# YukunXia/VLOAM-CMU-16833

Measured on AMD Instinct MI355X. Metric: scans/sec end-to-end odometry on 64x2048 cloud, higher is better.
Workload: dtype f32 points / f64 poses+residuals; 1 GPU; configs[2]: scanRegistration + laserOdometry + laserMapping scan-to-map ICP (voxel-hash local map, ~200 scans), synthetic HDL-64E 64x2048; sequences=1, map_warmup_sweeps=200, map_points_at_last_sweep=119454

## Files before the change

### vloam-cmu-16833_amd/csrc/map_inspect.hip

```cpp
#include <hip/hip_runtime.h>
#include <string.h>
#include <vector>
#include "map_kernels.h"

namespace vloam {

__global__ void k_map_error_fetch(MapFrame* fr, int clear_mask, int* out) { out[0] = atomicAnd(&fr->error, ~clear_mask); out[1] = fr->fallback_solves; }

vloam_status map_error(MapContext* m, int* e, int clear_mask, long long* fallback_solves) {
  *e = 0;
  if (fallback_solves) *fallback_solves = 0;
  for (int b = 0; b < m->se.B; b++) {
    const MapContext mb = m->for_session(b);
    int* d_out = mb.rebuild_n;
    VL_RAW_LAUNCH(k_map_error_fetch, dim3(1), dim3(1), 0, 0, mb.frame, clear_mask, d_out);
    int v[2] = {0, 0};
    if (hipMemcpy(v, d_out, sizeof(v), hipMemcpyDeviceToHost) != hipSuccess) return VLOAM_ERR_HIP;
    *e |= v[0];
    if (fallback_solves) *fallback_solves += v[1];
  }
  return VLOAM_OK;
}

vloam_status map_debug_get(MapContext* m0, int item, void* buf, long long cap, long long* n) {
  const MapContext msel = m0->for_session(m0->sel);
  const MapContext* m = &msel;
  if (item == 64) return copy_dev(m->state, sizeof(MapState), buf, cap, n);
  if (item == 65) return copy_dev(m->frame, sizeof(MapFrame), buf, cap, n);
  if (item == 66) return copy_dev(m->cube_cnt, sizeof(int) * 2 * kCubeNum, buf, cap, n);
  if (item == 67 || item == 68) {
    const VoxelTable& T = m->tab[item - 67];
    const size_t slots = (size_t)T.mask + 1;
    std::vector<VoxelRec> recs(slots);
    if (hipMemcpy(recs.data(), T.rec, slots * sizeof(VoxelRec), hipMemcpyDeviceToHost) != hipSuccess) return VLOAM_ERR_HIP;
    std::vector<unsigned> rows;
    for (size_t s = 0; s < slots; s++) {
      if (recs[s].key == 0 || recs[s].count == 0) continue;
      if ((recs[s].key >> 56) == 0 && (recs[s].count & (1 << 30))) continue;
      unsigned r[7];
      r[0] = (unsigned)(recs[s].key & 0xffffffffu); r[1] = (unsigned)(recs[s].key >> 32); r[2] = (unsigned)recs[s].count;
      memcpy(r + 3, &recs[s].sx, 16);
      rows.insert(rows.end(), r, r + 7);
    }
    if (n) *n = (long long)(rows.size() * 4);
    const size_t c = rows.size() * 4 < (size_t)cap ? rows.size() * 4 : (size_t)cap;
    if (buf && c) memcpy(buf, rows.data(), c);
    return VLOAM_OK;
  }
  if (item == 72) return copy_dev(m->ts_log, sizeof(long long) * 2048, buf, cap, n);
  if (item == 73) return copy_dev(m->cbox, sizeof(int4) * 2 * (size_t)m->factor_cap(), buf, cap, n);
  if (item == 71) return copy_dev(m->assoc_cyc, sizeof(long long) * 16, buf, cap, n);
  if (item == 69) {
    int out[12] = {0};
    for (int k = 0; k < 2; k++) if (hipMemcpy(out + 4 * k, m->tab[k].stats, 4 * sizeof(int), hipMemcpyDeviceToHost) != hipSuccess) return VLOAM_ERR_HIP;
    MapFrame fr;
    if (hipMemcpy(&fr, m->frame, sizeof(fr), hipMemcpyDeviceToHost) != hipSuccess) return VLOAM_ERR_HIP;
    out[8] = (int)m0->rebuilds; out[9] = fr.max_candidates; out[10] = fr.n_deferred[0] + fr.n_newraw[0]; out[11] = fr.n_deferred[1] + fr.n_newraw[1];
    if (n) *n = sizeof(out);
    if (buf) memcpy(buf, out, (size_t)cap < sizeof(out) ? (size_t)cap : sizeof(out));
    return VLOAM_OK;
  }
  const int outer = item / 16, k = item % 16;
  if (outer < 0 || outer > 1) return VLOAM_ERR_INVALID;
  const FactorTable& F = m->F[outer];
  switch (k) {
    case 0: return copy_dev(F.type, sizeof(int) * F.cap, buf, cap, n);
    case 1: return copy_dev(F.A, sizeof(double) * 3 * F.cap, buf, cap, n);
    case 2: return copy_dev(F.B, sizeof(double) * 3 * F.cap, buf, cap, n);
    case 3: return copy_dev(m->rec + outer, sizeof(LMRecord), buf, cap, n);
    case 4: return copy_dev(F.resid, sizeof(double) * 3 * F.cap, buf, cap, n);
    case 5: return copy_dev(F.p, sizeof(double) * 3 * F.cap, buf, cap, n);
  }
  return VLOAM_ERR_INVALID;
}

vloam_status map_counts(MapContext* m0, long long c[16]) {
  const MapContext msel = m0->for_session(m0->sel);
  const MapContext* m = &msel;
  MapState ms;
  MapFrame fr;
  LMRecord rec[2];
  if (hipMemcpy(&ms, m->state, sizeof(ms), hipMemcpyDeviceToHost) != hipSuccess) return VLOAM_ERR_HIP;
  if (hipMemcpy(&fr, m->frame, sizeof(fr), hipMemcpyDeviceToHost) != hipSuccess) return VLOAM_ERR_HIP;
  if (hipMemcpy(rec, m->rec, sizeof(rec), hipMemcpyDeviceToHost) != hipSuccess) return VLOAM_ERR_HIP;
  c[11] = ms.n_corner_stack; c[12] = ms.n_surf_stack;
  c[13] = fr.n_factors[1][0] + fr.n_factors[1][1];
  c[14] = ms.do_optimize ? (long long)(rec[0].n_evals + rec[1].n_evals) : 0;
  c[15] = ms.n_map_corner + ms.n_map_surf;
  return VLOAM_OK;
}

}
```

### vloam-cmu-16833_amd/csrc/map_kernels.h

```cpp
#pragma once
#include <hip/hip_runtime.h>
#include <vector>
#include "../../include/vloam_hip/c_api.h"
#include "sr_kernels.h"
#include "vloam_device.h"

namespace vloam {

constexpr int kCubeW = 21, kCubeH = 21, kCubeD = 11, kCubeNum = kCubeW * kCubeH * kCubeD;
constexpr int kStackCapCorner = 8192;
constexpr int kStackCapSurf = 24576;
constexpr int kMapFactorCap = kStackCapCorner + kStackCapSurf;
constexpr int kStackCapSurfStep = 8192, kStackCapSurfMax = 131072;
static_assert(kStackCapSurfMax <= (1 << 17), "the tier's raw-point arrival stamp keeps 17 bits of stack index (k_map_finalize_tier)");
constexpr int kPendCap = 16;
__host__ __device__ inline int vox_radix(float inv) { return (int)(50.0f * inv) + 4; }

struct __attribute__((aligned(32))) VoxelRec {
  unsigned long long key;
  float sx, sy, sz, si;
  int count;
  int pend_cnt;
};
static_assert(sizeof(VoxelRec) == 32, "one voxel, one half cache line");
// ... 67 lines not shown
  float4* out[2] = {nullptr, nullptr};
  PubHeader* hdr[2] = {nullptr, nullptr};
  float4* cloud[2] = {nullptr, nullptr};
  int* cloud_n[2] = {nullptr, nullptr};
  hipEvent_t ev_map[2] = {nullptr, nullptr}, ev_cloud[2] = {nullptr, nullptr};
  int map_seq = 0, cloud_seq = 0;
  int map_frame[2] = {-1, -1}, cloud_frame[2] = {-1, -1};
  int mapped = 0;
  void rebase(size_t o) {
    rbp(cnt, o); rbp(off, o); rbp(cur, o); rbp(keys, o); rbp(vals, o);
    for (int k = 0; k < 2; k++) { rbp(out[k], o); rbp(hdr[k], o); rbp(cloud[k], o); rbp(cloud_n[k], o); }
  }
};

struct MapGrow {
  int max_log2 = 28;
  int lg[2] = {0, 0};
  long long steps = 0;
  long long inc_rec[2] = {0, 0};
  long long inc_blk[2] = {0, 0};
  unsigned long long* progress = nullptr;
  long long step_at[2] = {-1, -1};
  static constexpr int kEvRing = 4;
  hipEvent_t ev_prog[kEvRing] = {};
  int failed_log2 = 0;
  struct Retired { void* p[3]; hipEvent_t ev; };
  std::vector<Retired> retired;
  std::vector<void*> leftover;
};

struct LocAux { int shift[3]; int si_error; double guess[7]; };
struct MapLocalize {
  char* base = nullptr;
  MapState* state = nullptr;
  MapFrame* frame = nullptr;
  LocAux* aux = nullptr;
  StackInfo* si = nullptr;
  FrameScalars* S = nullptr;
  float4* in[2] = {nullptr, nullptr};
  float4* stack[2] = {nullptr, nullptr};
  DsScratch ds[2];
  unsigned ds_gen = 0;
  FactorTable F[2];
  LMRecord* rec = nullptr;
  float4* nbr = nullptr;
  int4* cbox = nullptr;
  float4* ccand = nullptr;
  vloam_localize_result* result = nullptr;
};

struct CarveGeom {
  int rows, cols, n_sweeps, min_votes;
  float min_range, max_range, range_res;
  float elev_min, row_scale, col_scale;
  unsigned margin_q;
};
struct CarvePose { double R[9], t[3]; };
constexpr int kCarveMaxSweeps = 16, kCarveMaxPoints = 262144, kCarveMaxPixels = 1 << 20;
constexpr int kCarveCounters = 6;
struct CarveCounters { unsigned long long cnt[2][kCarveCounters]; unsigned long long n_removed; };
struct MapCarve { char* base = nullptr; size_t bytes = 0; };
struct MergeXf { double R[9], t[3]; int identity; };

struct MapArchive {
  char* base = nullptr;
  int* cnt = nullptr;
  vloam_map_archive_row* rows = nullptr;
  long long cap = 0;
  int frame = 0;
};

struct MapContext {
  MapState* state = nullptr;
  MapFrame* frame = nullptr;
  VoxelTable tab[2];
  int* cube_cnt = nullptr;
  DsScratch ds[2];
  unsigned ds_gen = 0;
  static constexpr int kSets = kBufferSets;
  float4* stack_sets[kSets][2] = {};
  StackInfo* stack_info[kSets] = {};
  float4* stack[2] = {nullptr, nullptr};
  float4* stack_map[2] = {nullptr, nullptr};
  int* touched[2] = {nullptr, nullptr};
  int* deferred[2] = {nullptr, nullptr};
  int* newraw[2] = {nullptr, nullptr};
  FactorTable F[2];
  LMRecord* rec = nullptr;
  int surf_cap = kStackCapSurf;
  int factor_cap() const { return kStackCapCorner + surf_cap; }
  bool tier() const { return surf_cap > kStackCapSurf; }
  float4* nbr = nullptr;
  int4* cbox = nullptr;
  float4* ccand = nullptr;
  VoxelRec* rebuild_tmp = nullptr;
  int rebuild_cap = 0;
  int* rebuild_n = nullptr;
  int* host_flags = nullptr;
  int rebuild_cooldown[kMaxBatch][2] = {};
  long long rebuilds = 0;
  MapGrow* grow = nullptr;
  Sess se;
  int sel = 0;
  MapContext for_session(int b) const {
    MapContext m = *this;
    const size_t off = (size_t)b * se.ss;
    rbp(m.state, off); rbp(m.frame, off); m.tab[0].rebase(off); m.tab[1].rebase(off); rbp(m.cube_cnt, off); m.ds[0].rebase(off); m.ds[1].rebase(off);
    for (int c = 0; c < kSets; c++) { rbp(m.stack_sets[c][0], off); rbp(m.stack_sets[c][1], off); rbp(m.stack_info[c], off); }
    for (int k = 0; k < 2; k++) { rbp(m.stack[k], off); rbp(m.stack_map[k], off); rbp(m.touched[k], off); rbp(m.deferred[k], off); rbp(m.newraw[k], off); m.F[k].rebase(off); }
    rbp(m.rec, off); rbp(m.nbr, off); rbp(m.cbox, off); rbp(m.ccand, off); rbp(m.registered, off); rbp(m.assoc_cyc, off); rbp(m.ts_log, off); rbp(m.rebuild_tmp, off); rbp(m.rebuild_n, off);
    if (m.host_flags) m.host_flags += 2 * b;
    m.pub.rebase(off);
    m.se.B = 1; m.sel = 0;
    return m;
  }
  MapLocalize* loc = nullptr;
  MapCarve* carve = nullptr;
  MapArchive* archive = nullptr;
  MapPub pub;
  float4* registered = nullptr;
  long long* assoc_cyc = nullptr;
  long long* ts_log = nullptr;
  int max_points = 0;
  float inv_leaf[2] = {0, 0};
};

vloam_status map_layout(MapContext* m, const vloam_config& cfg, Arena& A);
vloam_status map_init(MapContext* m, hipStream_t st);
vloam_status map_enqueue(MapContext* m, const vloam_config& cfg, hipStream_t st, const SRBuffers& cur, LOState* lo, double* traj_row14,
                         bool skip_frame, int set, ProfHook* ph, hipEvent_t done = nullptr);
vloam_status map_force_rebuild(MapContext* m, hipStream_t st);
vloam_status map_reclaim_enqueue(MapContext* m, hipStream_t st, int kind);
void map_destroy(MapContext* m);
vloam_status map_stack_enqueue(MapContext* m, hipStream_t st, const SRBuffers& cur, int set, ProfHook* ph, hipEvent_t done = nullptr);
vloam_status map_get_cloud(MapContext* m, hipStream_t st, int which, const SRBuffers& cur, float* xyzi4, int cap, int* n);
vloam_status map_export(MapContext* m, hipStream_t st, float* xyzi4, long long cap, long long* n);
vloam_status map_export_kind(MapContext* m, hipStream_t st, int kind, float* xyzi4, long long cap, long long* n);
bool map_publishes(const MapContext* m, bool skip_frame);
vloam_status map_publish_enqueue(MapContext* m, hipStream_t st, const float4* cloud, const FrameScalars* S, int frame, bool skip_frame, ProfHook* ph,
                                 hipEvent_t done);
vloam_status map_published_get(MapContext* m, int which, float* xyzi4, long long cap, long long* n, int* frame, void** d_ptr);
vloam_status map_error(MapContext* m, int* err_bits, int clear_mask = 0, long long* fallback_solves = nullptr);
vloam_status map_debug_get(MapContext* m, int item, void* buf, long long cap, long long* n);
vloam_status map_counts(MapContext* m, long long c[16]);
vloam_status map_query_enqueue(MapContext* m, hipStream_t st, int kind, int k, float radius, const void* d_xyz_pad4, int n, void* d_xyzi4, void* d_d2,
                               void* d_count);
vloam_status map_score_enqueue(MapContext* m, hipStream_t st, const void* d_corner, int n_corner, const void* d_surf, int n_surf, const int stride[2],
                               const float radius[2], const double* d_q4t3, int M, void* d_out);
vloam_status map_localize_alloc(MapContext* m, hipStream_t st);
void map_localize_free(MapContext* m);
vloam_status map_localize_enqueue(MapContext* m, hipStream_t st, const float4* corner, int n_corner, const float4* surf, int n_surf, int set,
                                  const double* row7, const double pose7[7], int pose_frame, vloam_localize_result* d_result);
void map_loc_prepare_launch(hipStream_t st, const MapContext* m, const StackInfo* si, const double* row7, const double pose7[7], int pose_frame);
void map_loc_finish_launch(hipStream_t st, const MapContext* m, vloam_localize_result* d_result);
void map_stack_enqueue_loc(MapContext* m, hipStream_t st, const float4* corner, const float4* surf);
vloam_status map_import_run(MapContext* m, hipStream_t st, const double pose7[7], const void* const cloud[2], const int n[2], bool host_clouds,
                            vloam_map_import_result* h_result);
vloam_status map_merge_run(MapContext* m, hipStream_t st, const MergeXf& X, const void* const cloud[2], const int n[2], bool host_clouds, bool apply,
                           bool place_start, vloam_map_merge_result* h_result);
inline bool map_window_never_placed(const MapState& s) { return s.sweep_no == 0 && s.centerCube[0] == 0 && s.centerCube[1] == 0 && s.centerCube[2] == 0; }
vloam_status map_carve_run(MapContext* m, int session, hipStream_t st, const CarveGeom& G, int kind_mask, const void* const* clouds, const int* n,
                           const CarvePose* poses, bool host_io, void* removed, long long cap, bool apply, CarveCounters* h_out);
void map_carve_free(MapContext* m);
vloam_status map_archive_alloc(MapContext* m, hipStream_t st, long long capacity_rows);
void map_archive_free(MapContext* m);
void map_archive_enqueue(const MapContext* m, hipStream_t st);
vloam_status map_force_grow(MapContext* m, hipStream_t st);
void map_grow_release(MapContext* m);
vloam_status map_grow_init(MapContext* m, hipStream_t st);
void map_grow_destroy(MapContext* m);
vloam_status map_grow_rehash(MapContext* m, hipStream_t st, int kind);
vloam_status map_grow_before_sweep(MapContext* m, hipStream_t st);
void map_grow_progress_enqueue(MapContext* m, hipStream_t st);
vloam_status map_ckpt_pack(MapContext* m, hipStream_t st, long long n_rec[2], VoxelRec** d_out, float ms[2]);
vloam_status map_ckpt_unpack(MapContext* m, hipStream_t st, const void* recs, const long long n_rec[2], float* ms);
int map_grow_restore_log2(const MapContext* m, int kind, long long live, long long blk);
vloam_status map_grow_restore(MapContext* m, hipStream_t st, const int lg[2], const long long live[2], const long long blk[2], long long mapped);

}
```

### vloam-cmu-16833_amd/csrc/map_kernels.hip

```cpp
#include <hip/hip_runtime.h>
#include <math.h>
#include <string.h>
#include <type_traits>
#include "lm_solve.h"
#include "map_kernels.h"
#include "map_device.h"
#include "map_table.h"
#include "map_move_dev.h"
#include "subwave.h"

namespace vloam {

__device__ void map_purge(const VoxelTable& T, const MapState* ms, int first, int stride) {
  const int cW = ms->cenW, cH = ms->cenH, cD = ms->cenD;
  int dead = 0;
  for (unsigned s = (unsigned)first; s <= T.mask; s += (unsigned)stride) {
    const RecVal v = rec_load(&T.rec[s]);
    if (v.key == 0 || v.count == 0) continue;
    int Ai, Aj, Ak;
    unpack_cube(v.key, &Ai, &Aj, &Ak);
    const int i = Ai + cW, j = Aj + cH, kk = Ak + cD;
    if (i < 0 || i >= kCubeW || j < 0 || j >= kCubeH || kk < 0 || kk >= kCubeD) { rec_store_value(&T.rec[s], make_float4(0.f, 0.f, 0.f, 0.f), 0, 0); dead++; }
  }
  if (dead) atomicAdd(&T.stats[1], dead);
// ... 327 lines not shown
      float4 cc[U];
#pragma unroll
      for (int u = 0; u < U; u++) {
        const int w = c0 + gl + u * G;
        cc[u] = make_float4(0.f, 0.f, 0.f, __uint_as_float(0xffffffffu));
        if (from_cache && act && w < total) cc[u] = ccand[(size_t)slot * kCandCache + w];
      }
#pragma unroll
      for (int u = 0; u < U; u++) {
        const unsigned tie = __float_as_uint(cc[u].w);
        const float d0 = q0 - cc[u].x, d1 = q1 - cc[u].y, d2 = q2 - cc[u].z;
        const u64 k = ((u64)__float_as_uint(d0 * d0 + d1 * d1 + d2 * d2) << 32) | tie;
        if (from_cache && tie != 0xffffffffu) { key_u[u] = k; px[u] = cc[u].x; py[u] = cc[u].y; pz[u] = cc[u].z; }
      }
    }
    if (dbg_cyc && c0 == 0) tp[4] = clock64() + ((int)key_u[0] & 0);
    select_rounds(act, c0 > 0);
    if (dbg_cyc && c0 == 0) tp[5] = clock64();
  }
  const int nraw = min(s_nraw[qi], kRawCap);
  const bool raw_overflow = s_nraw[qi] > kRawCap;
  if (__ballot(live && nraw > 0) != 0ull) {
    int total_raw = 0;
    for (c0 = 0;; c0 += CH) {
      const bool act = live && nraw > 0 && (c0 == 0 || c0 < total_raw);
      if (__ballot(act) == 0ull) break;
      reset_candidates();
      int produced = 0;
      for (int r0 = 0; __ballot(act && r0 < nraw) != 0ull; r0 += G) {
        const int r = r0 + gl;
        const int nr = (act && r < nraw) ? s_rawn[qi][r] : 0;
        const u64 vk = (act && r < nraw) ? s_rawk[qi][r] : 0ull;
        const int inc = grp_scan_incl<G>(nr);
        const int tot = grp_sum<G>(nr);
        int o = produced + inc - nr;
        for (int j = 1; j <= nr; j++, o++)
          if (o >= c0 && o < c0 + CH) s_cand[qi][o - c0] = key_with_seq(vk, j);
        produced += tot;
      }
      if (act) total_raw = produced;
      sw_lds_sync();
      ncand = act ? min(total_raw - c0, CH) : 0;
      probe_pair(std::integral_constant<int, 0>{});
      if constexpr (U > 2) { if (__ballot(2 * G < ncand) != 0ull) probe_pair(std::integral_constant<int, 2>{}); }
      select_rounds(act, true);
    }
  }
  if (outer == 0 && search && gl == 0) {
    cbox[2 * slot] = make_int4(blo0, bhi0, blo1, bhi1);
    cbox[2 * slot + 1] = make_int4(blo2, bhi2, (total <= kCandCache && !overflow && s_nraw[qi] == 0) ? total : -1, total);
  }
  if (live && gl < 5) {
    const u64 k4 = s_bestk[qi][4];
    const bool ok = k4 != ~0ull && __uint_as_float((unsigned)(k4 >> 32)) < 1.0f;
    float4 p = s_bestp[qi][gl];
    p.w = ok ? 1.0f : 0.0f;
    nbr[slot * 5 + gl] = p;
  }
  if (live && gl == 0 && total > kCandChunk) atomicMax(&fr->max_candidates, total);
  if (__ballot(chain_too_long || (live && overflow)) && lane == 0) atomicOr(&fr->error, kErrMapFull);
  if (__ballot(live && raw_overflow) && lane == 0) atomicOr(&fr->error, kErrMapDeferred);
  if (dbg_cyc && lane == 0) {
    tp[6] = clock64();
    if (tp[3] == 0) tp[3] = tp[2];
    if (tp[4] == 0) tp[4] = tp[3];
    for (int k = 0; k < 6; k++) atomicAdd((unsigned long long*)&dbg_cyc[outer * 8 + k], (unsigned long long)(tp[k + 1] - tp[k]));
    atomicAdd((unsigned long long*)&dbg_cyc[outer * 8 + 7], 1ull);
  }
}

#define VL_MAP_TIER 0
#define VL_MAP_KERNEL(name) name
#define VL_MAP_CAP_PARAM
#define VL_MAP_SURF_CAP kStackCapSurf
#define VL_MAP_FACTOR_CAP kMapFactorCap
#include "map_prepare_fit.inc.h"
#define VL_MAP_TIER 1
#define VL_MAP_KERNEL(name) name##_tier
#define VL_MAP_CAP_PARAM , int surf_cap
#define VL_MAP_SURF_CAP surf_cap
#define VL_MAP_FACTOR_CAP F.cap
#include "map_prepare_fit.inc.h"

__device__ void map_update(MapState* ms, double* traj_row14) {
  const double* q = ms->q_wodom_curr;
  const double n2 = q[0] * q[0] + q[1] * q[1] + q[2] * q[2] + q[3] * q[3];
  double qi[4] = {0, 0, 0, 0};
  if (n2 > 0.0) { qi[0] = -q[0] / n2; qi[1] = -q[1] / n2; qi[2] = -q[2] / n2; qi[3] = q[3] / n2; }
  double r[4], t[3];
  dquat_mul(ms->parameters, qi, r);
  for (int k = 0; k < 4; k++) ms->q_wmap_wodom[k] = r[k];
  dquat_rot(ms->q_wmap_wodom, ms->t_wodom_curr, t);
  for (int k = 0; k < 3; k++) ms->t_wmap_wodom[k] = ms->parameters[4 + k] - t[k];
  if (traj_row14) for (int k = 0; k < 7; k++) traj_row14[7 + k] = ms->parameters[k];
}

__device__ bool map_put_raw_point(const VoxelTable& T, u64 voxel_key, int seq, float4 p, int stamp) {
  const u64 key = key_with_seq(voxel_key, seq);
  unsigned s = (unsigned)mix64(key) & T.mask;
  for (int probe = 0; probe < kMaxProbe; probe++, s = (s + 1) & T.mask) {
    const u64 old = atomicCAS(&T.rec[s].key, 0ull, key);
    if (old == 0ull || old == key) {
      if (old == 0ull) atomicAdd(&T.stats[0], 1);
      rec_store_value(&T.rec[s], p, 1, stamp);
      return true;
    }
  }
  return false;
}
__device__ void map_drop_raw_points(const VoxelTable& T, u64 voxel_key, int n) {
  int dead = 0;
  for (int seq = 1; seq <= min(n, 255); seq++) {
    const u64 key = key_with_seq(voxel_key, seq);
    unsigned s = (unsigned)mix64(key) & T.mask;
    for (int probe = 0; probe < kMaxProbe; probe++, s = (s + 1) & T.mask) {
      const u64 k = T.rec[s].key;
      if (k == 0ull) break;
      if (k == key) { rec_store_value(&T.rec[s], make_float4(0.f, 0.f, 0.f, 0.f), 0, 0); dead++; break; }
    }
  }
  if (dead) atomicAdd(&T.stats[1], dead);
}

template <bool TIER>
__device__ __forceinline__ void map_insert_body(const float4* __restrict__ stack0, const float4* __restrict__ stack1,
                                                float4* __restrict__ smap0, float4* __restrict__ smap1, VoxelTable T0, VoxelTable T1,
                                                float inv0, float inv1, MapState* ms, MapFrame* fr, int* __restrict__ touched0,
                                                int* __restrict__ touched1, int* __restrict__ deferred0, int* __restrict__ deferred1,
                                                double* traj_row14, size_t ss, int surf_cap) {
  VL_SESSION(ss); RB(stack0); RB(stack1); RB(smap0); RB(smap1); T0.rebase(so_); T1.rebase(so_); RB(ms); RB(fr); RB(touched0); RB(touched1);
  RB(deferred0); RB(deferred1); RB(traj_row14);
  if (blockIdx.x == 0 && blockIdx.y == 0 && threadIdx.x == 0) map_update(ms, traj_row14);
  const int kind = blockIdx.y;
  const VoxelTable T = kind ? T1 : T0;
  const float inv = kind ? inv1 : inv0;
  const float4* stack = kind ? stack1 : stack0;
  float4* smap = kind ? smap1 : smap0;
  int* touched = kind ? touched1 : touched0;
  (void)deferred0; (void)deferred1;
  const int n = kind ? ms->n_surf_stack : ms->n_corner_stack;
  const int cap = kind ? (TIER ? surf_cap : kStackCapSurf) : kStackCapCorner;
  const int lane = threadIdx.x & 63;
  const int i_first = blockIdx.x * 256 + threadIdx.x;
  const float4 p_first = stack[i_first < cap ? i_first : 0];
  for (int i0 = blockIdx.x * 256 + (threadIdx.x & ~63); i0 < n; i0 += gridDim.x * 256) {
    const int i = i0 + lane;
    auto insert_point = [&]() -> int {
      if (i >= n) return -1;
      const float4 p = associate_to_map(i == i_first ? p_first : stack[i], ms->parameters, ms->parameters + 4);
      smap[i] = p;
      const int Ai = cube_abs((double)p.x), Aj = cube_abs((double)p.y), Ak = cube_abs((double)p.z);
      const int wi = Ai + ms->cenW, wj = Aj + ms->cenH, wk = Ak + ms->cenD;
      if (wi < 0 || wi >= kCubeW || wj < 0 || wj >= kCubeH || wk < 0 || wk >= kCubeD) return -1;
      const int lx = (int)floorf(p.x * inv) - cube_voxel_base(Ai, inv), ly = (int)floorf(p.y * inv) - cube_voxel_base(Aj, inv),
                lz = (int)floorf(p.z * inv) - cube_voxel_base(Ak, inv);
      if ((unsigned)lx > (unsigned)kVoxMax || (unsigned)ly > (unsigned)kVoxMax || (unsigned)lz > (unsigned)kVoxMax || !cube_in_key_range(Ai, Aj, Ak)) { atomicOr(&fr->error, kErrMapFull); return -1; }
      const u64 key = pack_key(Ai, Aj, Ak, lx, ly, lz);
      unsigned s = (unsigned)mix64(key) & T.mask;
      for (int probe = 0; probe < kMaxProbe; probe++, s = (s + 1) & T.mask) {
        const u64 old = atomicCAS(&T.rec[s].key, 0ull, key);
        if (old == 0ull || old == key) {
          if (old == 0ull) {
            atomicAdd(&T.stats[0], 1);
            if (!map_publish_block(T, Ai, Aj, Ak, lx, ly, lz)) atomicOr(&fr->error, kErrMapFull);
          }
          const int pos = atomicAdd(&T.rec[s].pend_cnt, 1);
          if (pos < kPendCap) T.pend[(size_t)s * kPendCap + pos] = i; else atomicOr(&fr->error, kErrMapFull);
          return pos == 0 ? (int)s : -1;
        }
      }
      atomicOr(&fr->error, kErrMapFull);
      return -1;
    };
    const int first = insert_point();
    const u64 tm = __ballot(first >= 0);
    if (tm != 0ull) {
      const int leader = __ffsll((long long)tm) - 1;
      int base = 0;
      if (lane == leader) base = atomicAdd(&fr->n_touched[kind], __popcll(tm));
      base = __shfl(base, leader);
      if (first >= 0) {
        const int tpos = base + __popcll(tm & ((1ull << lane) - 1ull));
        if (tpos < cap) touched[tpos] = first; else atomicOr(&fr->error, kErrMapFull);
      }
    }
  }
}
#define VL_MAP_INSERT_PARAMS const float4* __restrict__ stack0, const float4* __restrict__ stack1, float4* __restrict__ smap0, float4* __restrict__ smap1, \
    VoxelTable T0, VoxelTable T1, float inv0, float inv1, MapState* ms, MapFrame* fr, int* __restrict__ touched0, int* __restrict__ touched1,      \
    int* __restrict__ deferred0, int* __restrict__ deferred1, double* traj_row14, size_t ss
#define VL_MAP_INSERT_ARGS stack0, stack1, smap0, smap1, T0, T1, inv0, inv1, ms, fr, touched0, touched1, deferred0, deferred1, traj_row14, ss
__global__ __launch_bounds__(256) void k_map_insert(VL_MAP_INSERT_PARAMS) { map_insert_body<false>(VL_MAP_INSERT_ARGS, kStackCapSurf); }
__global__ __launch_bounds__(256) void k_map_insert_tier(VL_MAP_INSERT_PARAMS, int surf_cap) { map_insert_body<true>(VL_MAP_INSERT_ARGS, surf_cap); }
#undef VL_MAP_INSERT_PARAMS
#undef VL_MAP_INSERT_ARGS

template <bool TIER>
__device__ __forceinline__ void map_finalize_body(const float4* __restrict__ smap0, const float4* __restrict__ smap1, VoxelTable T0,
                                                  VoxelTable T1, MapState* ms, MapFrame* fr,
                                                  const int* __restrict__ touched0, const int* __restrict__ touched1,
                                                  int* __restrict__ deferred0, int* __restrict__ deferred1, int* __restrict__ newraw0,
                                                  int* __restrict__ newraw1, int* __restrict__ cube_cnt, int* host_flags, long long* ts_log, size_t ss,
                                                  int surf_cap) {
  VL_SESSION(ss); RB(smap0); RB(smap1); T0.rebase(so_); T1.rebase(so_); RB(ms); RB(fr); RB(touched0); RB(touched1); RB(deferred0); RB(deferred1);
  RB(newraw0); RB(newraw1); RB(cube_cnt); RB(ts_log);
  if (ts_log && blockIdx.x == 0 && blockIdx.y == 0 && threadIdx.x == 0) ts_log[2 * ((ms->sweep_no - 1) & 1023) + 1] = (long long)wall_clock64();
  if (host_flags) host_flags += 2 * blockIdx.z;
  const int kind = blockIdx.y;
  const VoxelTable T = kind ? T1 : T0;
  const float4* smap = kind ? smap1 : smap0;
  const int* touched = kind ? touched1 : touched0;
  const int cap = kind ? (TIER ? surf_cap : kStackCapSurf) : kStackCapCorner;
  const int t = blockIdx.x * 256 + threadIdx.x;
  const int s_spec = touched[t < cap ? t : 0];
  const int nt = min(fr->n_touched[kind], cap);
  const int cI = ms->centerCube[0], cJ = ms->centerCube[1], cK = ms->centerCube[2];
  int* deferred = kind ? deferred1 : deferred0;
  int* newraw = kind ? newraw1 : newraw0;
  if (t < nt) {
    const int s = s_spec;
    int idx[kPendCap];
    const RecVal rv = rec_load(&T.rec[s]);
    const int np = min(rv.pend_cnt, kPendCap);
    for (int a = 0; a < np; a++) idx[a] = T.pend[(size_t)s * kPendCap + a];
    for (int a = 1; a < np; a++) {
      const int v = idx[a];
      int c = a - 1;
      while (c >= 0 && idx[c] > v) { idx[c + 1] = idx[c]; c--; }
      idx[c + 1] = v;
    }
    const int n_old = rec_n(rv.count);
    const bool was_raw = rec_raw(rv.count);
    float4 acc = n_old > 0 ? rv.sum : make_float4(0.f, 0.f, 0.f, 0.f);
    int Ai, Aj, Ak;
    unpack_cube(rv.key, &Ai, &Aj, &Ak);
    const int wi = Ai + ms->cenW, wj = Aj + ms->cenH, wk = Ak + ms->cenD;
    int* cube_n = &cube_cnt[kind * kCubeNum + wi + kCubeW * wj + kCubeW * kCubeH * wk];
    const bool valid = abs(wi - cI) <= 2 && abs(wj - cJ) <= 2 && abs(wk - cK) <= 1;
    if (valid) {
      if (was_raw) map_drop_raw_points(T, rv.key, n_old);
      for (int a = 0; a < np; a++) { const float4 p = smap[idx[a]]; acc.x += p.x; acc.y += p.y; acc.z += p.z; acc.w += p.w; }
      const float nn = (float)(n_old + np);
      acc.x = acc.x / nn; acc.y = acc.y / nn; acc.z = acc.z / nn; acc.w = acc.w / nn;
      const int held = was_raw ? n_old : (n_old > 0 ? 1 : 0);
      if (held != 1) atomicAdd(cube_n, 1 - held);
      rec_store_value(&T.rec[s], acc, 1, 0);
    } else {
      int seq = n_old;
      bool overflow = false;
      if (!was_raw) {
        if (n_old == 1 && !map_put_raw_point(T, rv.key, 1, rv.sum, 0)) overflow = true;
        const int dpos = atomicAdd(&fr->n_newraw[kind], 1);
        if (dpos < cap) newraw[dpos] = s; else atomicOr(&fr->error, kErrMapFull);
        atomicAdd(&ms->deferred, 1);
      }
      for (int a = 0; a < np; a++) {
        const float4 p = smap[idx[a]];
        acc.x += p.x; acc.y += p.y; acc.z += p.z; acc.w += p.w;
        seq++;
        const int stamp = TIER ? (int)(((unsigned)ms->sweep_no & 0x7fffu) << 17) | idx[a] : ((ms->sweep_no & 0x3ffff) << 14) | idx[a];
        if (seq > 255 || !map_put_raw_point(T, rv.key, seq, p, stamp)) overflow = true;
      }
      if (overflow) atomicOr(&fr->error, kErrMapDeferred);
      atomicAdd(cube_n, np);
      rec_store_value(&T.rec[s], acc, min(seq, 0xffff) | kRecRaw, 0);
    }
  }
  if (blockIdx.x == 0) {
    __shared__ int s_wcnt[4], s_out;
    const int nd = min(fr->n_deferred[kind], cap);
    if (threadIdx.x == 0) s_out = 0;
    __syncthreads();
    for (int base = 0; base < nd; base += 256) {
      const int d = base + threadIdx.x;
      int s = d < nd ? deferred[d] : -1;
      if (s >= 0) {
        const RecVal dv = rec_load(&T.rec[s]);
        int Ai, Aj, Ak;
        unpack_cube(dv.key, &Ai, &Aj, &Ak);
        const int wi = Ai + ms->cenW, wj = Aj + ms->cenH, wk = Ak + ms->cenD;
        const bool in_window = wi >= 0 && wi < kCubeW && wj >= 0 && wj < kCubeH && wk >= 0 && wk < kCubeD;
        if (!in_window || dv.count == 0) s = -1;
        else if (abs(wi - cI) <= 2 && abs(wj - cJ) <= 2 && abs(wk - cK) <= 1) {
          if (dv.pend_cnt == 0 && rec_raw(dv.count)) {
            const int n = rec_n(dv.count);
            map_drop_raw_points(T, dv.key, n);
            float4 a = dv.sum; const float nn = (float)n;
            a.x /= nn; a.y /= nn; a.z /= nn; a.w /= nn;
            rec_store_value(&T.rec[s], a, 1, 0);
            if (n != 1) atomicAdd(&cube_cnt[kind * kCubeNum + wi + kCubeW * wj + kCubeW * kCubeH * wk], 1 - n);
          }
          s = -1;
        }
      }
      const unsigned long long keep = __ballot(s >= 0);
      if ((threadIdx.x & 63) == 0) s_wcnt[threadIdx.x >> 6] = __popcll(keep);
      __syncthreads();
      int o = s_out;
      for (int w = 0; w < (int)(threadIdx.x >> 6); w++) o += s_wcnt[w];
      if (s >= 0) deferred[o + __popcll(keep & ((1ull << (threadIdx.x & 63)) - 1ull))] = s;
      __syncthreads();
      if (threadIdx.x == 0) s_out += s_wcnt[0] + s_wcnt[1] + s_wcnt[2] + s_wcnt[3];
      __syncthreads();
    }
    if (threadIdx.x == 0) fr->n_deferred[kind] = s_out;
  }
  if (fr->rolled) map_purge(T, ms, blockIdx.x * 256 + threadIdx.x, gridDim.x * 256);
  if (blockIdx.x == 0 && threadIdx.x == 0) {
    const long long slots = (long long)T.mask + 1;
    const int keys = T.stats[0], dead = T.stats[1];
    if ((long long)(keys - dead) * 10 > slots * 6 || (long long)T.stats[2] * 10 > ((long long)T.bslots_mask + 1) * 6) atomicOr(&fr->error, kErrMapFull);
    if (host_flags) {
      const int want = ((long long)dead * 8 > slots || (long long)keys * 2 > slots) && dead > 0 ? 1 : 0;
      __hip_atomic_store(&host_flags[kind], want, __ATOMIC_RELAXED, __HIP_MEMORY_SCOPE_SYSTEM);
    }
  }
}
#define VL_MAP_FINALIZE_PARAMS const float4* __restrict__ smap0, const float4* __restrict__ smap1, VoxelTable T0, VoxelTable T1, MapState* ms, MapFrame* fr, \
    const int* __restrict__ touched0, const int* __restrict__ touched1, int* __restrict__ deferred0, int* __restrict__ deferred1,                      \
    int* __restrict__ newraw0, int* __restrict__ newraw1, int* __restrict__ cube_cnt, int* host_flags, long long* ts_log, size_t ss
#define VL_MAP_FINALIZE_ARGS smap0, smap1, T0, T1, ms, fr, touched0, touched1, deferred0, deferred1, newraw0, newraw1, cube_cnt, host_flags, ts_log, ss
__global__ __launch_bounds__(256) void k_map_finalize(VL_MAP_FINALIZE_PARAMS) { map_finalize_body<false>(VL_MAP_FINALIZE_ARGS, kStackCapSurf); }
__global__ __launch_bounds__(256) void k_map_finalize_tier(VL_MAP_FINALIZE_PARAMS, int surf_cap) { map_finalize_body<true>(VL_MAP_FINALIZE_ARGS, surf_cap); }
#undef VL_MAP_FINALIZE_PARAMS
#undef VL_MAP_FINALIZE_ARGS

__global__ __launch_bounds__(256) void k_map_rebuild_gather(VoxelTable T, VoxelRec* __restrict__ tmp, int cap, int* n_tmp, MapFrame* fr, int kind) {
  if (blockIdx.x == 0 && threadIdx.x == 0) map_move_begin(T, fr, kind);
  for (unsigned s = blockIdx.x * 256 + threadIdx.x; s <= T.mask; s += gridDim.x * 256) {
    const RecVal v = rec_load(&T.rec[s]);
    if (!rec_live(v)) continue;
    const int o = atomicAdd(n_tmp, 1);
    if (o < cap) rec_store_all(&tmp[o], v);
    else atomicOr(&fr->error, kErrMapFull);
  }
}
__global__ __launch_bounds__(256) void k_map_rebuild_insert(VoxelTable T, const VoxelRec* __restrict__ tmp, int cap, int* n_tmp, MapFrame* fr, int kind,
                                                            int* __restrict__ deferred, int deferred_cap, int* host_flags) {
  const int n = min(*n_tmp, cap);
  for (int e = blockIdx.x * 256 + threadIdx.x; e < n; e += gridDim.x * 256)
    map_reinsert(T, rec_load(&tmp[e]), fr, kind, deferred, deferred_cap);
  if (blockIdx.x == 0 && threadIdx.x == 0) {
    T.stats[0] = n;
    if (host_flags) __hip_atomic_store(&host_flags[kind], 0, __ATOMIC_RELAXED, __HIP_MEMORY_SCOPE_SYSTEM);
  }
}

vloam_status map_layout(MapContext* m, const vloam_config& cfg, Arena& A) {
  bool ok = true;
  ok = ok && A.take(&m->state, 1) && A.take(&m->frame, 1) && A.take(&m->cube_cnt, 2 * (size_t)kCubeNum);
  const int lg = cfg.map_capacity_log2 < 10 ? 10 : (cfg.map_capacity_log2 > 28 ? 28 : cfg.map_capacity_log2);
  const size_t slots = (size_t)1 << lg;
  for (int k = 0; k < 2 && ok; k++) {
    VoxelTable& T = m->tab[k];
    if (m->grow) { T.rec = nullptr; T.pend = nullptr; T.blk = nullptr; ok = ok && A.take(&T.stats, 4); }
    else ok = ok && A.take(&T.rec, slots) && A.take(&T.pend, slots * kPendCap) && A.take(&T.stats, 4);
    T.mask = (unsigned)(slots - 1);
    const size_t bslots = slots / 2;
    if (!m->grow) ok = ok && A.take(&T.blk, bslots);
    T.bslots_mask = (unsigned)(bslots - 1);
    DsScratch& D = m->ds[k];
    if (k == 0) for (int c = 0; c < MapContext::kSets; c++) ok = ok && A.take(&m->stack_info[c], 1);
    D.stack_cap = k ? m->surf_cap : kStackCapCorner;
    ok = ok && A.take(&D.region, (size_t)kDsMaxBins * kDsBinCap) && A.take(&D.over, (size_t)cfg.max_points) && A.take(&D.tmp, (size_t)cfg.max_points) &&
         A.take(&D.sorted, (size_t)cfg.max_points) && A.take(&D.splitters, (size_t)kDsMaxBins) && A.take(&D.cursor, (size_t)kDsMaxBins + 4) &&
         A.take(&D.done, (size_t)kDsMaxBins);
    for (int c = 0; c < MapContext::kSets; c++) ok = ok && A.take(&m->stack_sets[c][k], (size_t)D.stack_cap);
    m->stack[k] = m->stack_sets[0][k];
    ok = ok && A.take(&m->stack_map[k], (size_t)D.stack_cap) && A.take(&m->touched[k], (size_t)D.stack_cap) && A.take(&m->deferred[k], (size_t)D.stack_cap) &&
         A.take(&m->newraw[k], (size_t)D.stack_cap);
    FactorTable& F = m->F[k];
    F.cap = m->factor_cap();
    ok = ok && A.take(&F.type, (size_t)F.cap) && A.take(&F.p, 3 * (size_t)F.cap) && A.take(&F.A, 3 * (size_t)F.cap) && A.take(&F.B, 3 * (size_t)F.cap) &&
         A.take(&F.resid, 3 * (size_t)F.cap) && A.take(&F.ctype, (size_t)F.cap) && A.take(&F.cslot, (size_t)F.cap) && A.take(&F.cpack, 11 * (size_t)F.cap) && A.take(&F.dg, 8 * (size_t)F.cap) &&
         A.take(&F.rowcnt, (size_t)F.cap / 64 + 1);
    if (m->tier()) F.rowmask = nullptr;
    else ok = ok && A.take(&F.rowmask, (size_t)F.cap / 64 + 2);
    F.gsync = nullptr;
    F.err = ok ? &m->frame->error : nullptr;
    F.fallbacks = ok ? &m->frame->fallback_solves : nullptr;
    F.host_degraded = nullptr;
    F.gen = 0; F.spin_limit = 1 << 18;
  }
  ok = ok && A.take(&m->rec, 2) && A.take(&m->nbr, 5 * (size_t)m->factor_cap());
  ok = ok && A.take(&m->cbox, 2 * (size_t)m->factor_cap()) && A.take(&m->ccand, (size_t)m->factor_cap() * kCandCache);
  m->rebuild_cap = m->grow ? 0 : (int)(slots / 2);
  if (m->grow) { m->rebuild_tmp = nullptr; m->grow->lg[0] = m->grow->lg[1] = lg; ok = ok && A.take(&m->rebuild_n, 2); }
  else ok = ok && A.take(&m->rebuild_tmp, (size_t)m->rebuild_cap) && A.take(&m->rebuild_n, 2);
  ok = ok && A.take(&m->registered, (size_t)cfg.max_points) && A.take(&m->assoc_cyc, 16) && A.take(&m->ts_log, 2048);
  MapPub& P = m->pub;
  if (P.pub_number > 0) {
    ok = ok && A.take(&P.cnt, (size_t)kPubBuckets) && A.take(&P.off, (size_t)kPubBuckets + 1) && A.take(&P.cur, (size_t)kPubBuckets) &&
         A.take(&P.keys, (size_t)P.cap) && A.take(&P.vals, (size_t)P.cap);
    for (int k = 0; k < 2; k++) ok = ok && A.take(&P.out[k], (size_t)P.cap) && A.take(&P.hdr[k], 1);
  }
  if (P.cloud_on) for (int k = 0; k < 2; k++) ok = ok && A.take(&P.cloud[k], (size_t)cfg.max_points) && A.take(&P.cloud_n[k], 1);
  if (!ok) return VLOAM_ERR_HIP;
  m->max_points = cfg.max_points;
  m->inv_leaf[0] = 1.0f / cfg.mapping_line_resolution;
  m->inv_leaf[1] = 1.0f / cfg.mapping_plane_resolution;
  return VLOAM_OK;
}
// ... 154 lines not shown
```

### vloam-cmu-16833_amd/csrc/map_table.h

```cpp
#pragma once
#include <hip/hip_runtime.h>
#include "map_kernels.h"

namespace vloam {

typedef unsigned long long u64;

__device__ __forceinline__ u64 mix64(u64 x) {
  x ^= x >> 33; x *= 0xff51afd7ed558ccdull; x ^= x >> 33; x *= 0xc4ceb9fe1a85ec53ull; x ^= x >> 33;
  return x;
}

constexpr int kCubeOffXY = 512, kCubeOffZ = 128;
constexpr int kVoxBits = 9, kVoxMax = (1 << kVoxBits) - 1;
__device__ __forceinline__ u64 pack_key(int Ai, int Aj, int Ak, int lx, int ly, int lz) {
  return ((u64)(unsigned)(Ai + kCubeOffXY) << 45) | ((u64)(unsigned)(Aj + kCubeOffXY) << 35) | ((u64)(unsigned)(Ak + kCubeOffZ) << 27) |
         ((u64)(unsigned)lx << (2 * kVoxBits)) | ((u64)(unsigned)ly << kVoxBits) | (u64)(unsigned)lz;
}
__device__ __forceinline__ void unpack_cube(u64 k, int* Ai, int* Aj, int* Ak) {
  *Ai = (int)((k >> 45) & 0x3ff) - kCubeOffXY; *Aj = (int)((k >> 35) & 0x3ff) - kCubeOffXY; *Ak = (int)((k >> 27) & 0xff) - kCubeOffZ;
}
__device__ __forceinline__ int key_lx(u64 k) { return (int)((k >> (2 * kVoxBits)) & kVoxMax); }
__device__ __forceinline__ int key_ly(u64 k) { return (int)((k >> kVoxBits) & kVoxMax); }
__device__ __forceinline__ int key_lz(u64 k) { return (int)(k & kVoxMax); }
__device__ __forceinline__ bool cube_in_key_range(int Ai, int Aj, int Ak) {
  return Ai >= -kCubeOffXY && Ai < kCubeOffXY && Aj >= -kCubeOffXY && Aj < kCubeOffXY && Ak >= -kCubeOffZ && Ak < kCubeOffZ;
}
__device__ __forceinline__ int key_seq(u64 k) { return (int)(k >> 56); }
__device__ __forceinline__ u64 key_with_seq(u64 k, int seq) { return (k & 0x00ffffffffffffffull) | ((u64)(unsigned)seq << 56); }
constexpr int kRecRaw = 1 << 30;
__device__ __forceinline__ int rec_n(int count) { return count & 0xffff; }
__device__ __forceinline__ bool rec_raw(int count) { return (count & kRecRaw) != 0; }

struct RecVal { u64 key; float4 sum; int count, pend_cnt; };
__device__ __forceinline__ RecVal rec_load(const VoxelRec* r) {
  const uint4 a = reinterpret_cast<const uint4*>(r)[0], b = reinterpret_cast<const uint4*>(r)[1];
  RecVal v;
  v.key = (u64)a.x | ((u64)a.y << 32);
  v.sum = make_float4(__uint_as_float(a.z), __uint_as_float(a.w), __uint_as_float(b.x), __uint_as_float(b.y));
  v.count = (int)b.z; v.pend_cnt = (int)b.w;
  return v;
}
__device__ __forceinline__ bool rec_live(const RecVal& v) { return v.key != 0ull && v.count != 0; }
__device__ __forceinline__ void rec_store_value(VoxelRec* r, float4 sum, int count, int pend_cnt) {
  reinterpret_cast<float2*>(r)[1] = make_float2(sum.x, sum.y);
  reinterpret_cast<uint4*>(r)[1] = make_uint4(__float_as_uint(sum.z), __float_as_uint(sum.w), (unsigned)count, (unsigned)pend_cnt);
}
__device__ __forceinline__ void rec_store_all(VoxelRec* r, const RecVal& v) {
  uint4* o = reinterpret_cast<uint4*>(r);
  o[0] = make_uint4((unsigned)v.key, (unsigned)(v.key >> 32), __float_as_uint(v.sum.x), __float_as_uint(v.sum.y));
  o[1] = make_uint4(__float_as_uint(v.sum.z), __float_as_uint(v.sum.w), (unsigned)v.count, key_seq(v.key) ? (unsigned)v.pend_cnt : 0u);
}

__device__ __forceinline__ bool rec_find(const VoxelTable& T, u64 key, RecVal* out, unsigned* slot, bool* chain_too_long) {
  unsigned s = (unsigned)mix64(key) & T.mask;
  for (int probe = 0; probe < kMaxProbe; probe++, s = (s + 1) & T.mask) {
    const RecVal v = rec_load(&T.rec[s]);
    if (v.key == 0ull) return false;
    if (v.key == key) { *out = v; if (slot) *slot = s; return true; }
  }
  *chain_too_long = true;
  return false;
}

__device__ __forceinline__ float4 rec_point(const RecVal& v) {
  const int n = key_seq(v.key) ? 1 : rec_n(v.count);
  const float nn = (float)n;
  return make_float4(n > 1 ? v.sum.x / nn : v.sum.x, n > 1 ? v.sum.y / nn : v.sum.y, n > 1 ? v.sum.z / nn : v.sum.z, n > 1 ? v.sum.w / nn : v.sum.w);
}
__device__ __forceinline__ u64 rec_order_key(const RecVal& v, int cube_index, int kind) {
  const u64 lx = (u64)key_lx(v.key), ly = (u64)key_ly(v.key), lz = (u64)key_lz(v.key);
  const bool tail = key_seq(v.key) != 0 && v.pend_cnt != 0;
  return ((u64)cube_index << 50) | ((u64)kind << 49) | ((u64)(tail ? 1 : 0) << 48) | (tail ? (u64)(unsigned)v.pend_cnt : ((lz << (2 * kVoxBits)) | (ly << kVoxBits) | lx));
}

__device__ bool map_publish_block(const VoxelTable& T, int Ai, int Aj, int Ak, int lx, int ly, int lz) {
  const u64 bkey = pack_key(Ai, Aj, Ak, lx >> 2, ly >> 2, lz >> 2) | (1ull << 63);
  unsigned bs = (unsigned)mix64(bkey) & T.bslots_mask;
  for (int bp = 0; bp < kMaxProbe; bp++, bs = (bs + 1) & T.bslots_mask) {
    const u64 bold = atomicCAS(&T.blk[bs].x, 0ull, bkey);
    if (bold == 0ull || bold == bkey) {
      if (bold == 0ull) atomicAdd(&T.stats[2], 1);
      atomicOr(&T.blk[bs].y, 1ull << (((lz & 3) << 4) | ((ly & 3) << 2) | (lx & 3)));
      return true;
    }
  }
  return false;
}

}
```

Baseline: 6798 scans/s.

## Carry first point index in touched list and drop per-thread pending sort

```diff
diff --git a/vloam-cmu-16833_amd/csrc/map_inspect.hip b/vloam-cmu-16833_amd/csrc/map_inspect.hip
--- a/vloam-cmu-16833_amd/csrc/map_inspect.hip
+++ b/vloam-cmu-16833_amd/csrc/map_inspect.hip
@@ -50,6 +50,7 @@
   if (item == 72) return copy_dev(m->ts_log, sizeof(long long) * 2048, buf, cap, n);
   if (item == 73) return copy_dev(m->cbox, sizeof(int4) * 2 * (size_t)m->factor_cap(), buf, cap, n);
   if (item == 71) return copy_dev(m->assoc_cyc, sizeof(long long) * 16, buf, cap, n);
+  if (item == 75) return map_update_cycles_get(buf, cap, n);
   if (item == 69) {
     int out[12] = {0};
     for (int k = 0; k < 2; k++) if (hipMemcpy(out + 4 * k, m->tab[k].stats, 4 * sizeof(int), hipMemcpyDeviceToHost) != hipSuccess) return VLOAM_ERR_HIP;
diff --git a/vloam-cmu-16833_amd/csrc/map_kernels.h b/vloam-cmu-16833_amd/csrc/map_kernels.h
--- a/vloam-cmu-16833_amd/csrc/map_kernels.h
+++ b/vloam-cmu-16833_amd/csrc/map_kernels.h
@@ -173,7 +173,7 @@
   StackInfo* stack_info[kSets] = {};
   float4* stack[2] = {nullptr, nullptr};
   float4* stack_map[2] = {nullptr, nullptr};
-  int* touched[2] = {nullptr, nullptr};
+  int2* touched[2] = {nullptr, nullptr};
   int* deferred[2] = {nullptr, nullptr};
   int* newraw[2] = {nullptr, nullptr};
   FactorTable F[2];
@@ -233,6 +233,7 @@
 vloam_status map_published_get(MapContext* m, int which, float* xyzi4, long long cap, long long* n, int* frame, void** d_ptr);
 vloam_status map_error(MapContext* m, int* err_bits, int clear_mask = 0, long long* fallback_solves = nullptr);
 vloam_status map_debug_get(MapContext* m, int item, void* buf, long long cap, long long* n);
+vloam_status map_update_cycles_get(void* buf, long long cap, long long* n);
 vloam_status map_counts(MapContext* m, long long c[16]);
 vloam_status map_query_enqueue(MapContext* m, hipStream_t st, int kind, int k, float radius, const void* d_xyz_pad4, int n, void* d_xyzi4, void* d_d2,
                                void* d_count);
diff --git a/vloam-cmu-16833_amd/csrc/map_kernels.hip b/vloam-cmu-16833_amd/csrc/map_kernels.hip
--- a/vloam-cmu-16833_amd/csrc/map_kernels.hip
+++ b/vloam-cmu-16833_amd/csrc/map_kernels.hip
@@ -433,6 +433,32 @@
 #define VL_MAP_FACTOR_CAP F.cap
 #include "map_prepare_fit.inc.h"
 
+#ifdef VLOAM_MAP_STAMPS
+__device__ unsigned long long g_upd_cyc[32];
+#define UPD_STAMPS(n) long long ts_[n] = {}
+#define UPD_STAMP(k, dep) do { asm volatile("" ::"v"((int)(dep))); ts_[k] = (long long)clock64(); } while (0)
+template <int N>
+__device__ __forceinline__ void upd_stamps_flush(long long (&ts)[N], int base, int count_at) {
+  for (int k = 1; k < N; k++) if (ts[k] == 0) ts[k] = ts[k - 1];
+  for (int k = 0; k < N; k++)
+    for (int o = 32; o > 0; o >>= 1) { const long long e = __shfl_xor(ts[k], o); ts[k] = e > ts[k] ? e : ts[k]; }
+  if ((threadIdx.x & 63) == 0)
+    for (int k = 0; k + 1 < N; k++) atomicAdd(&g_upd_cyc[base + k], (unsigned long long)(ts[k + 1] - ts[k]));
+  if ((threadIdx.x & 63) == 0) atomicAdd(&g_upd_cyc[count_at], 1ull);
+}
+vloam_status map_update_cycles_get(void* buf, long long cap, long long* n) {
+  unsigned long long host[32];
+  if (hipMemcpyFromSymbol(host, HIP_SYMBOL(g_upd_cyc), sizeof(host)) != hipSuccess) return VLOAM_ERR_HIP;
+  if (n) *n = (long long)sizeof(host);
+  if (buf && cap > 0) memcpy(buf, host, (size_t)cap < sizeof(host) ? (size_t)cap : sizeof(host));
+  return VLOAM_OK;
+}
+#else
+#define UPD_STAMPS(n) ((void)0)
+#define UPD_STAMP(k, dep) ((void)0)
+vloam_status map_update_cycles_get(void*, long long, long long*) { return VLOAM_ERR_INVALID; }
+#endif
+
 __device__ void map_update(MapState* ms, double* traj_row14) {
   const double* q = ms->q_wodom_curr;
   const double n2 = q[0] * q[0] + q[1] * q[1] + q[2] * q[2] + q[3] * q[3];
@@ -476,8 +502,8 @@
 template <bool TIER>
 __device__ __forceinline__ void map_insert_body(const float4* __restrict__ stack0, const float4* __restrict__ stack1,
                                                 float4* __restrict__ smap0, float4* __restrict__ smap1, VoxelTable T0, VoxelTable T1,
-                                                float inv0, float inv1, MapState* ms, MapFrame* fr, int* __restrict__ touched0,
-                                                int* __restrict__ touched1, int* __restrict__ deferred0, int* __restrict__ deferred1,
+                                                float inv0, float inv1, MapState* ms, MapFrame* fr, int2* __restrict__ touched0,
+                                                int2* __restrict__ touched1, int* __restrict__ deferred0, int* __restrict__ deferred1,
                                                 double* traj_row14, size_t ss, int surf_cap) {
   VL_SESSION(ss); RB(stack0); RB(stack1); RB(smap0); RB(smap1); T0.rebase(so_); T1.rebase(so_); RB(ms); RB(fr); RB(touched0); RB(touched1);
   RB(deferred0); RB(deferred1); RB(traj_row14);
@@ -487,7 +513,7 @@
   const float inv = kind ? inv1 : inv0;
   const float4* stack = kind ? stack1 : stack0;
   float4* smap = kind ? smap1 : smap0;
-  int* touched = kind ? touched1 : touched0;
+  int2* touched = kind ? touched1 : touched0;
   (void)deferred0; (void)deferred1;
   const int n = kind ? ms->n_surf_stack : ms->n_corner_stack;
   const int cap = kind ? (TIER ? surf_cap : kStackCapSurf) : kStackCapCorner;
@@ -496,10 +522,14 @@
   const float4 p_first = stack[i_first < cap ? i_first : 0];
   for (int i0 = blockIdx.x * 256 + (threadIdx.x & ~63); i0 < n; i0 += gridDim.x * 256) {
     const int i = i0 + lane;
+    UPD_STAMPS(6);
+    UPD_STAMP(0, 0);
+    bool new_key = false, new_blk = false;
     auto insert_point = [&]() -> int {
       if (i >= n) return -1;
       const float4 p = associate_to_map(i == i_first ? p_first : stack[i], ms->parameters, ms->parameters + 4);
       smap[i] = p;
+      UPD_STAMP(1, __float_as_int(p.x));
       const int Ai = cube_abs((double)p.x), Aj = cube_abs((double)p.y), Ak = cube_abs((double)p.z);
       const int wi = Ai + ms->cenW, wj = Aj + ms->cenH, wk = Ak + ms->cenD;
       if (wi < 0 || wi >= kCubeW || wj < 0 || wj >= kCubeH || wk < 0 || wk >= kCubeD) return -1;
@@ -511,12 +541,17 @@
       for (int probe = 0; probe < kMaxProbe; probe++, s = (s + 1) & T.mask) {
         const u64 old = atomicCAS(&T.rec[s].key, 0ull, key);
         if (old == 0ull || old == key) {
+          UPD_STAMP(2, old);
           if (old == 0ull) {
-            atomicAdd(&T.stats[0], 1);
-            if (!map_publish_block(T, Ai, Aj, Ak, lx, ly, lz)) atomicOr(&fr->error, kErrMapFull);
+            new_key = true;
+            const bool published = map_publish_block_uncounted(T, Ai, Aj, Ak, lx, ly, lz, &new_blk);
+            if (!published) atomicOr(&fr->error, kErrMapFull);
+            UPD_STAMP(3, published);
           }
           const int pos = atomicAdd(&T.rec[s].pend_cnt, 1);
-          if (pos < kPendCap) T.pend[(size_t)s * kPendCap + pos] = i; else atomicOr(&fr->error, kErrMapFull);
+          UPD_STAMP(4, pos);
+          if (pos >= kPendCap) atomicOr(&fr->error, kErrMapFull);
+          else if (pos > 0) T.pend[(size_t)s * kPendCap + pos] = i;
           return pos == 0 ? (int)s : -1;
         }
       }
@@ -524,7 +559,9 @@
       return -1;
     };
     const int first = insert_point();
-    const u64 tm = __ballot(first >= 0);
+    const u64 tm = __ballot(first >= 0), km = __ballot(new_key), bm = __ballot(new_blk);
+    if (lane == 0 && km != 0ull) atomicAdd(&T.stats[0], __popcll(km));
+    if (lane == 0 && bm != 0ull) atomicAdd(&T.stats[2], __popcll(bm));
     if (tm != 0ull) {
       const int leader = __ffsll((long long)tm) - 1;
       int base = 0;
@@ -532,13 +569,17 @@
       base = __shfl(base, leader);
       if (first >= 0) {
         const int tpos = base + __popcll(tm & ((1ull << lane) - 1ull));
-        if (tpos < cap) touched[tpos] = first; else atomicOr(&fr->error, kErrMapFull);
-      }
-    }
+        if (tpos < cap) touched[tpos] = make_int2(first, i); else atomicOr(&fr->error, kErrMapFull);
+      }
+      UPD_STAMP(5, base);
+    }
+#ifdef VLOAM_MAP_STAMPS
+    upd_stamps_flush(ts_, 0, 7);
+#endif
   }
 }
 #define VL_MAP_INSERT_PARAMS const float4* __restrict__ stack0, const float4* __restrict__ stack1, float4* __restrict__ smap0, float4* __restrict__ smap1, \
-    VoxelTable T0, VoxelTable T1, float inv0, float inv1, MapState* ms, MapFrame* fr, int* __restrict__ touched0, int* __restrict__ touched1,      \
+    VoxelTable T0, VoxelTable T1, float inv0, float inv1, MapState* ms, MapFrame* fr, int2* __restrict__ touched0, int2* __restrict__ touched1,    \
     int* __restrict__ deferred0, int* __restrict__ deferred1, double* traj_row14, size_t ss
 #define VL_MAP_INSERT_ARGS stack0, stack1, smap0, smap1, T0, T1, inv0, inv1, ms, fr, touched0, touched1, deferred0, deferred1, traj_row14, ss
 __global__ __launch_bounds__(256) void k_map_insert(VL_MAP_INSERT_PARAMS) { map_insert_body<false>(VL_MAP_INSERT_ARGS, kStackCapSurf); }
@@ -549,7 +590,7 @@
 template <bool TIER>
 __device__ __forceinline__ void map_finalize_body(const float4* __restrict__ smap0, const float4* __restrict__ smap1, VoxelTable T0,
                                                   VoxelTable T1, MapState* ms, MapFrame* fr,
-                                                  const int* __restrict__ touched0, const int* __restrict__ touched1,
+                                                  const int2* __restrict__ touched0, const int2* __restrict__ touched1,
                                                   int* __restrict__ deferred0, int* __restrict__ deferred1, int* __restrict__ newraw0,
                                                   int* __restrict__ newraw1, int* __restrict__ cube_cnt, int* host_flags, long long* ts_log, size_t ss,
                                                   int surf_cap) {
@@ -560,26 +601,33 @@
   const int kind = blockIdx.y;
   const VoxelTable T = kind ? T1 : T0;
   const float4* smap = kind ? smap1 : smap0;
-  const int* touched = kind ? touched1 : touched0;
+  const int2* touched = kind ? touched1 : touched0;
   const int cap = kind ? (TIER ? surf_cap : kStackCapSurf) : kStackCapCorner;
   const int t = blockIdx.x * 256 + threadIdx.x;
-  const int s_spec = touched[t < cap ? t : 0];
+  UPD_STAMPS(9);
+  UPD_STAMP(0, 0);
+  const int2 e_spec = touched[t < cap ? t : 0];
   const int nt = min(fr->n_touched[kind], cap);
   const int cI = ms->centerCube[0], cJ = ms->centerCube[1], cK = ms->centerCube[2];
+  const int rolled = fr->rolled;
+  const int nd = blockIdx.x == 0 ? min(fr->n_deferred[kind], cap) : 0;
+  UPD_STAMP(1, e_spec.x + nt + cI + cJ + cK + rolled + nd);
   int* deferred = kind ? deferred1 : deferred0;
   int* newraw = kind ? newraw1 : newraw0;
   if (t < nt) {
-    const int s = s_spec;
-    int idx[kPendCap];
+    const int s = e_spec.x, i_first = e_spec.y;
     const RecVal rv = rec_load(&T.rec[s]);
+    const float4 p_first = smap[i_first];
+    UPD_STAMP(2, rv.count);
     const int np = min(rv.pend_cnt, kPendCap);
-    for (int a = 0; a < np; a++) idx[a] = T.pend[(size_t)s * kPendCap + a];
-    for (int a = 1; a < np; a++) {
-      const int v = idx[a];
-      int c = a - 1;
-      while (c >= 0 && idx[c] > v) { idx[c + 1] = idx[c]; c--; }
-      idx[c + 1] = v;
-    }
+    const int* __restrict__ pend = T.pend + (size_t)s * kPendCap;
+    auto next_index = [&](int last) -> int {
+      if (np == 1) return i_first;
+      int cur = i_first > last ? i_first : INT_MAX;
+      for (int b = 1; b < np; b++) { const int v = pend[b]; cur = (v > last && v < cur) ? v : cur; }
+      return cur != INT_MAX ? cur : i_first;
+    };
+    UPD_STAMP(3, np > 1 ? pend[1] : 0);
     const int n_old = rec_n(rv.count);
     const bool was_raw = rec_raw(rv.count);
     float4 acc = n_old > 0 ? rv.sum : make_float4(0.f, 0.f, 0.f, 0.f);
@@ -590,12 +638,19 @@
     const bool valid = abs(wi - cI) <= 2 && abs(wj - cJ) <= 2 && abs(wk - cK) <= 1;
     if (valid) {
       if (was_raw) map_drop_raw_points(T, rv.key, n_old);
-      for (int a = 0; a < np; a++) { const float4 p = smap[idx[a]]; acc.x += p.x; acc.y += p.y; acc.z += p.z; acc.w += p.w; }
+      for (int a = 0, last = -1; a < np; a++) {
+        const int cur = next_index(last);
+        const float4 p = cur == i_first ? p_first : smap[cur];
+        acc.x += p.x; acc.y += p.y; acc.z += p.z; acc.w += p.w;
+        last = cur;
+      }
+      UPD_STAMP(4, __float_as_int(acc.x));
       const float nn = (float)(n_old + np);
       acc.x = acc.x / nn; acc.y = acc.y / nn; acc.z = acc.z / nn; acc.w = acc.w / nn;
       const int held = was_raw ? n_old : (n_old > 0 ? 1 : 0);
       if (held != 1) atomicAdd(cube_n, 1 - held);
       rec_store_value(&T.rec[s], acc, 1, 0);
+      UPD_STAMP(5, 0);
     } else {
       int seq = n_old;
       bool overflow = false;
@@ -605,11 +660,13 @@
         if (dpos < cap) newraw[dpos] = s; else atomicOr(&fr->error, kErrMapFull);
         atomicAdd(&ms->deferred, 1);
       }
-      for (int a = 0; a < np; a++) {
-        const float4 p = smap[idx[a]];
+      for (int a = 0, last = -1; a < np; a++) {
+        const int cur = next_index(last);
+        const float4 p = cur == i_first ? p_first : smap[cur];
+        last = cur;
         acc.x += p.x; acc.y += p.y; acc.z += p.z; acc.w += p.w;
         seq++;
-        const int stamp = TIER ? (int)(((unsigned)ms->sweep_no & 0x7fffu) << 17) | idx[a] : ((ms->sweep_no & 0x3ffff) << 14) | idx[a];
+        const int stamp = TIER ? (int)(((unsigned)ms->sweep_no & 0x7fffu) << 17) | cur : ((ms->sweep_no & 0x3ffff) << 14) | cur;
         if (seq > 255 || !map_put_raw_point(T, rv.key, seq, p, stamp)) overflow = true;
       }
       if (overflow) atomicOr(&fr->error, kErrMapDeferred);
@@ -617,9 +674,8 @@
       rec_store_value(&T.rec[s], acc, min(seq, 0xffff) | kRecRaw, 0);
     }
   }
-  if (blockIdx.x == 0) {
+  if (nd > 0) {
     __shared__ int s_wcnt[4], s_out;
-    const int nd = min(fr->n_deferred[kind], cap);
     if (threadIdx.x == 0) s_out = 0;
     __syncthreads();
     for (int base = 0; base < nd; base += 256) {
@@ -655,8 +711,10 @@
       __syncthreads();
     }
     if (threadIdx.x == 0) fr->n_deferred[kind] = s_out;
-  }
-  if (fr->rolled) map_purge(T, ms, blockIdx.x * 256 + threadIdx.x, gridDim.x * 256);
+    UPD_STAMP(6, nd);
+  }
+  UPD_STAMP(7, rolled);
+  if (rolled) map_purge(T, ms, blockIdx.x * 256 + threadIdx.x, gridDim.x * 256);
   if (blockIdx.x == 0 && threadIdx.x == 0) {
     const long long slots = (long long)T.mask + 1;
     const int keys = T.stats[0], dead = T.stats[1];
@@ -666,9 +724,14 @@
       __hip_atomic_store(&host_flags[kind], want, __ATOMIC_RELAXED, __HIP_MEMORY_SCOPE_SYSTEM);
     }
   }
+#ifdef VLOAM_MAP_STAMPS
+  UPD_STAMP(8, 0);
+  if (__ballot(t < nt) != 0ull) upd_stamps_flush(ts_, 8, 16);
+  else if ((threadIdx.x & 63) == 0) { atomicAdd(&g_upd_cyc[17], (unsigned long long)(ts_[8] - ts_[0])); atomicAdd(&g_upd_cyc[18], 1ull); }
+#endif
 }
 #define VL_MAP_FINALIZE_PARAMS const float4* __restrict__ smap0, const float4* __restrict__ smap1, VoxelTable T0, VoxelTable T1, MapState* ms, MapFrame* fr, \
-    const int* __restrict__ touched0, const int* __restrict__ touched1, int* __restrict__ deferred0, int* __restrict__ deferred1,                      \
+    const int2* __restrict__ touched0, const int2* __restrict__ touched1, int* __restrict__ deferred0, int* __restrict__ deferred1,                      \
     int* __restrict__ newraw0, int* __restrict__ newraw1, int* __restrict__ cube_cnt, int* host_flags, long long* ts_log, size_t ss
 #define VL_MAP_FINALIZE_ARGS smap0, smap1, T0, T1, ms, fr, touched0, touched1, deferred0, deferred1, newraw0, newraw1, cube_cnt, host_flags, ts_log, ss
 __global__ __launch_bounds__(256) void k_map_finalize(VL_MAP_FINALIZE_PARAMS) { map_finalize_body<false>(VL_MAP_FINALIZE_ARGS, kStackCapSurf); }
diff --git a/vloam-cmu-16833_amd/csrc/map_table.h b/vloam-cmu-16833_amd/csrc/map_table.h
--- a/vloam-cmu-16833_amd/csrc/map_table.h
+++ b/vloam-cmu-16833_amd/csrc/map_table.h
@@ -74,18 +74,25 @@
   return ((u64)cube_index << 50) | ((u64)kind << 49) | ((u64)(tail ? 1 : 0) << 48) | (tail ? (u64)(unsigned)v.pend_cnt : ((lz << (2 * kVoxBits)) | (ly << kVoxBits) | lx));
 }
 
-__device__ bool map_publish_block(const VoxelTable& T, int Ai, int Aj, int Ak, int lx, int ly, int lz) {
+__device__ __forceinline__ bool map_publish_block_uncounted(const VoxelTable& T, int Ai, int Aj, int Ak, int lx, int ly, int lz, bool* fresh) {
   const u64 bkey = pack_key(Ai, Aj, Ak, lx >> 2, ly >> 2, lz >> 2) | (1ull << 63);
   unsigned bs = (unsigned)mix64(bkey) & T.bslots_mask;
   for (int bp = 0; bp < kMaxProbe; bp++, bs = (bs + 1) & T.bslots_mask) {
     const u64 bold = atomicCAS(&T.blk[bs].x, 0ull, bkey);
     if (bold == 0ull || bold == bkey) {
-      if (bold == 0ull) atomicAdd(&T.stats[2], 1);
+      *fresh = bold == 0ull;
       atomicOr(&T.blk[bs].y, 1ull << (((lz & 3) << 4) | ((ly & 3) << 2) | (lx & 3)));
       return true;
     }
   }
+  *fresh = false;
   return false;
+}
+__device__ bool map_publish_block(const VoxelTable& T, int Ai, int Aj, int Ak, int lx, int ly, int lz) {
+  bool fresh;
+  const bool ok = map_publish_block_uncounted(T, Ai, Aj, Ak, lx, ly, lz, &fresh);
+  if (fresh) atomicAdd(&T.stats[2], 1);
+  return ok;
 }
 
 }
```

New measurement: 6648 scans/s. 0.978x the previous value.
